# kingjosephm/GAN

Measured on AMD Instinct MI355X. Metric: Pix2Pix train_step images/sec at 256x256, higher is better.
Workload: dtype bf16; 1 GPU; Pix2Pix 256x256 bf16 batch=16/GPU train_step (G fwd, D fwd real+fake, losses, dgrad+wgrad, Adam); global_batch=16, img_size=256, channels=1, parallelism=dp1, hipgraph=True

## Files before the change

gan_amd/csrc/host_util.cpp:

```cpp
#include <nmmintrin.h>
#include <stddef.h>
#include <stdint.h>
#include <string.h>
#include "../../include/gan_amd.h"

extern "C" uint32_t gan_crc32c(uint32_t crc, const void* data, size_t n) {
  const unsigned char* p = (const unsigned char*)data;
  uint64_t c = crc ^ 0xffffffffu;
  while (n && ((uintptr_t)p & 7)) { c = _mm_crc32_u8((uint32_t)c, *p++); --n; }
  while (n >= 8) { uint64_t v; memcpy(&v, p, 8); c = _mm_crc32_u64(c, v); p += 8; n -= 8; }
  while (n) { c = _mm_crc32_u8((uint32_t)c, *p++); --n; }
  return (uint32_t)c ^ 0xffffffffu;
}

#include <atomic>
namespace {
struct Opt { const char* key; std::atomic<int> value; };
Opt g_opts[] = {
    {"conv.big_tiles", {1}},
    {"conv.q128", {55}},
    {"conv.q256n", {80}},
    {"conv.big_min_blocks", {64}},
    {"conv.tall64", {1}},
    {"conv.lean_epilogue", {1}},
    {"conv.tap_share", {7}},
    {"conv.pingpong", {1}},
    {"conv.parity_patch", {1}},
    {"conv.parity_patch_max_n", {64}},
    {"conv.parity_patch_min_blocks", {192}},
    {"conv.split_target", {256}},
    {"conv.split_target_skinny", {1024}},
    {"conv.split_target_big", {256}},
    {"conv.split_target_256", {128}},
    {"conv.split_min_ktiles", {4}},
    {"conv.split_max", {64}},
    {"conv.bwd_fuse_tile", {1}},
    {"conv.stack", {0}},
    {"conv.stack_blocks", {256}},
    {"conv.reduce_stats_rg", {16}},
    {"conv.own_max_kb", {192}},
    {"conv.own_max_rows", {16}},
    {"conv.skn512_min_rows", {0}},
    {"conv.norm_fuse", {1}},
    {"conv.thin_fused", {1}},
    {"conv.thin_k_blocks", {2048}},
    {"conv.thin", {7}},
    {"wgrad.tile256", {0}},
    {"wgrad.pingpong", {1}},
    {"wgrad.row_table", {1}},
    {"wgrad.pingpong_min_rows", {0}},
    {"wgrad.pingpong_128", {1}},
    {"wgrad.pingpong_min_gflop", {30}},
    {"wgrad.split_target", {512}},
    {"wgrad.fold_split_target", {512}},
    {"wgrad.reduce_adam_min_params", {1 << 20}},
    {"wgrad.reduce_adam", {1}},
    {"wgrad.adam_halves_max_rows", {0}},
    {"wgrad.dead_taps", {1}},
    {"norm.fin_in_apply", {0}},
    {"diag.launch_log", {0}},
};
Opt* find_opt(const char* key) {
  if (!key) return nullptr;
  for (Opt& o : g_opts)
    if (!strcmp(o.key, key)) return &o;
  return nullptr;
}
}

int gan_opt(const char* key) {
  Opt* o = find_opt(key);
  return o ? o->value.load(std::memory_order_relaxed) : 0;
}
#include <mutex>
#include <vector>
namespace {
std::atomic<int> g_log_on{0};
std::mutex g_log_mu;
std::vector<const void*> g_log;
}
void gan_launch_note(const void* kernel_host_fn) {
  if (!g_log_on.load(std::memory_order_relaxed)) return;
  std::lock_guard<std::mutex> lk(g_log_mu);
  g_log.push_back(kernel_host_fn);
}
size_t gan_launch_log_ptrs(const void** out, size_t cap) {
  std::lock_guard<std::mutex> lk(g_log_mu);
  for (size_t i = 0; i < g_log.size() && i < cap; ++i) out[i] = g_log[i];
  return g_log.size();
}

extern "C" int gan_set_option(const char* key, int32_t value) {
  Opt* o = find_opt(key);
  if (!o) return GAN_E_ARG;
  o->value.store(value, std::memory_order_relaxed);
  if (!strcmp(key, "diag.launch_log")) {
    std::lock_guard<std::mutex> lk(g_log_mu);
    if (value) g_log.clear();
    g_log_on.store(value ? 1 : 0, std::memory_order_relaxed);
  }
  return 0;
}
extern "C" int gan_get_option(const char* key, int32_t* value) {
  Opt* o = find_opt(key);
  if (!o || !value) return GAN_E_ARG;
  *value = o->value.load(std::memory_order_relaxed);
  return 0;
}
```

gan_amd/csrc/thin.hip:

```cpp
#include "common.h"
#include "conv_params.h"
#include <stdlib.h>
#include <type_traits>

typedef __attribute__((ext_vector_type(8))) short s16x8;
#ifndef THIN_ZS
#define THIN_ZS 20
#endif


struct ThinKParams {
  const void* x; const void* w; void* y; const float* bias;
  int Hs, Ws, xpitch, Hg, Wg, M, S, dy0, dstep, Wrows, ypitch, act, tiles;
  float slope;
  FastDiv divWg, divHg;
};

template <typename T, int ACT>
__global__ __launch_bounds__(256) void conv_thin_k_kernel(const ThinKParams p) {
  const int lane = threadIdx.x & 63, wave = threadIdx.x >> 6;
  const int n = lane & 15, q = lane >> 4;
  const int cbase = blockIdx.y * 64;
  uint4 wf[4][4];
#pragma unroll
  for (int ct = 0; ct < 4; ++ct) {
    const int ch = cbase + (ct >> 1) * 32 + (n >> 2) * 8 + (ct & 1) * 4 + (n & 3);
#pragma unroll
    for (int s = 0; s < 4; ++s) wf[ct][s] = *(const uint4*)((const T*)p.w + ((size_t)(s * 4 + q) * p.Wrows + ch) * 8);
  }
  float bv[2][8];
#pragma unroll
  for (int pr = 0; pr < 2; ++pr)
#pragma unroll
    for (int i = 0; i < 8; ++i) bv[pr][i] = p.bias ? p.bias[cbase + pr * 32 + q * 8 + i] : 0.f;

  for (int tile = blockIdx.x * 4 + wave; tile < p.tiles; tile += gridDim.x * 4) {
    const int m = tile * 16 + n;
    const unsigned t = fdiv((unsigned)m, p.divWg);
    const int gx = m - (int)t * p.Wg;
    const unsigned img = fdiv(t, p.divHg);
    const int gy = (int)t - (int)img * p.Hg;
    const bool rowok = m < p.M;
    const int sx = gx * p.S + p.dy0 + q * p.dstep;
    uint4 xf[4];
#pragma unroll
    for (int s = 0; s < 4; ++s) {
      const int sy = gy * p.S + p.dy0 + s * p.dstep;
      xf[s] = make_uint4(0, 0, 0, 0);
      if (rowok && (unsigned)sy < (unsigned)p.Hs && (unsigned)sx < (unsigned)p.Ws)
        xf[s] = *(const uint4*)((const T*)p.x + ((size_t)(img * p.Hs + sy) * p.Ws + sx) * p.xpitch);
    }
    f32x4 acc[4];
#pragma unroll
    for (int ct = 0; ct < 4; ++ct) {
      acc[ct] = f32x4{0.f, 0.f, 0.f, 0.f};
#pragma unroll
      for (int s = 0; s < 4; ++s) acc[ct] = mma16<T>(wf[ct][s], xf[s], acc[ct]);
    }
    if (rowok) {
      T* yp = (T*)p.y + ((size_t)(img * p.Hg + gy) * p.Wg + gx) * p.ypitch + cbase + q * 8;
#pragma unroll
      for (int pr = 0; pr < 2; ++pr) {
        float v[8];
#pragma unroll
        for (int i = 0; i < 4; ++i) {
          if constexpr (ACT >= 0) {
            v[i] = act_c<ACT>(acc[2 * pr][i] + bv[pr][i], p.slope);
            v[4 + i] = act_c<ACT>(acc[2 * pr + 1][i] + bv[pr][4 + i], p.slope);
          } else {
            v[i] = apply_act(acc[2 * pr][i] + bv[pr][i], p.act, p.slope);
            v[4 + i] = apply_act(acc[2 * pr + 1][i] + bv[pr][4 + i], p.act, p.slope);
          }
        }
        *(uint4*)(yp + pr * 32) = pack16<T>(v);
      }
    }
  }
}

struct ThinNParams {
  const void* x; const void* w; float* z;
  int Mx, xpitch, Cin, Wrows, CO, tiles;
};

template <typename T, int KS>
__global__ __launch_bounds__(256) void conv_thin_n_kernel(const ThinNParams p) {
  extern __shared__ __attribute__((aligned(16))) unsigned char smem[];
  uint4* wl = (uint4*)smem;
  const int lane = threadIdx.x & 63, wave = threadIdx.x >> 6;
  const int n = lane & 15, q = lane >> 4;
  for (int e = threadIdx.x; e < p.CO * KS * 64; e += 256) {
    const int l = e & 63, s = (e >> 6) % KS, c = (e >> 6) / KS;
    wl[e] = *(const uint4*)((const T*)p.w + ((size_t)(l & 15) * p.Wrows + c) * p.Cin + s * 32 + (l >> 4) * 8);
  }
  __syncthreads();
  for (int tile = blockIdx.x * 4 + wave; tile < p.tiles; tile += gridDim.x * 4) {
    const int pix = tile * 16 + n;
    const bool ok = pix < p.Mx;
    uint4 xf[KS];
    const T* xp = (const T*)p.x + (size_t)pix * p.xpitch + q * 8;
#pragma unroll
    for (int s = 0; s < KS; ++s) xf[s] = ok ? *(const uint4*)(xp + s * 32) : make_uint4(0, 0, 0, 0);
    for (int c = 0; c < p.CO; ++c) {
      f32x4 acc = f32x4{0.f, 0.f, 0.f, 0.f};
#pragma unroll
      for (int s = 0; s < KS; ++s) acc = mma16<T>(wl[(c * KS + s) * 64 + lane], xf[s], acc);
      if (ok) *(f32x4*)(p.z + ((size_t)pix * p.CO + c) * 16 + q * 4) = acc;
    }
  }
}

struct Col2imParams {
  const float* z; void* y; const float* bias;
  int Hs, Ws, Ho, Wo, CO, ypitch, out_f32, act, parity, S, dy0, dstep, f16;
  float slope;
  long long total;
  FastDiv divWo, divHo;
};

__global__ __launch_bounds__(256) void conv_thin_col2im_kernel(const Col2imParams p) {
  const long long idx = (long long)blockIdx.x * 256 + threadIdx.x;
  if (idx >= p.total) return;
  const unsigned t = fdiv((unsigned)idx, p.divWo);
  const int X = (int)idx - (int)t * p.Wo;
  const unsigned img = fdiv(t, p.divHo);
  const int Y = (int)t - (int)img * p.Ho;
  int iy[4], ky[4], ix[4], kx[4], ny, nx;
  if (p.parity) {
    ny = nx = 2;
    const int py = Y & 1, gy = Y >> 1, px = X & 1, gx = X >> 1;
#pragma unroll
    for (int a = 0; a < 2; ++a) {
      iy[a] = gy + py - a; ky[a] = 1 - py + 2 * a;
      ix[a] = gx + px - a; kx[a] = 1 - px + 2 * a;
    }
  } else {
    ny = nx = 4;
#pragma unroll
    for (int a = 0; a < 4; ++a) {
      iy[a] = Y * p.S + p.dy0 + a * p.dstep; ky[a] = a;
      ix[a] = X * p.S + p.dy0 + a * p.dstep; kx[a] = a;
    }
  }
  float acc[6] = {0.f, 0.f, 0.f, 0.f, 0.f, 0.f};
  for (int a = 0; a < ny; ++a) {
    if ((unsigned)iy[a] >= (unsigned)p.Hs) continue;
    for (int b = 0; b < nx; ++b) {
      if ((unsigned)ix[b] >= (unsigned)p.Ws) continue;
      const float* zp = p.z + ((size_t)(img * p.Hs + iy[a]) * p.Ws + ix[b]) * p.CO * 16 + ky[a] * 4 + kx[b];
#pragma unroll
      for (int c = 0; c < 6; ++c)
        if (c < p.CO) acc[c] += zp[c * 16];
    }
  }
  const size_t o = ((size_t)(img * p.Ho + Y) * p.Wo + X) * p.ypitch;
#pragma unroll
  for (int c = 0; c < 6; ++c) {
    if (c >= p.CO) break;
    float v = acc[c] + (p.bias ? p.bias[c] : 0.f);
    v = apply_act(v, p.act, p.slope);
    if (p.out_f32) ((float*)p.y)[o + c] = v;
    else if (p.f16) ((f16_t*)p.y)[o + c] = (f16_t)v;
    else ((bf16_t*)p.y)[o + c] = (bf16_t)v;
  }
}

struct ThinNFusedParams {
  const void* x; const void* w; void* y; const float* bias;
  int Hs, Ws, xpitch, Cin, Wrows, CO;
  int Ho, Wo, ypitch, out_f32, act, f16;
  float slope;
  int tilesY, tilesX;
};

template <typename T, int KS, bool PARITY, int TH, int TW>
__global__ __launch_bounds__(256) void conv_thin_n_fused_kernel(const ThinNFusedParams p) {
  constexpr int HB = 1, HA = PARITY ? 1 : 2;
  constexpr int SH = TH + HB + HA, SW = TW + HB + HA, NPX = SH * SW, NT = (NPX + 15) / 16;
  extern __shared__ __attribute__((aligned(16))) unsigned char smem[];
  uint4* wl = (uint4*)smem;
  constexpr int ZS = THIN_ZS;
  float* zl = (float*)(smem + (size_t)p.CO * KS * 1024);
  const int lane = threadIdx.x & 63, wave = threadIdx.x >> 6;
  const int n = lane & 15, q = lane >> 4;
  int b = blockIdx.x;
  const int tx = b % p.tilesX; b /= p.tilesX;
  const int ty = b % p.tilesY; const int img = b / p.tilesY;
  const int y0 = ty * TH - HB, x0 = tx * TW - HB;
  for (int e = threadIdx.x; e < p.CO * KS * 64; e += 256) {
    const int l = e & 63, s = (e >> 6) % KS, c = (e >> 6) / KS;
    wl[e] = *(const uint4*)((const T*)p.w + ((size_t)(l & 15) * p.Wrows + c) * p.Cin + s * 32 + (l >> 4) * 8);
  }
  __syncthreads();
  for (int tile = wave; tile < NT; tile += 4) {
    const int e = tile * 16 + n;
    const int hy = e / SW, hx = e - hy * SW;
    const int sy = y0 + hy, sx = x0 + hx;
    const bool ok = e < NPX && (unsigned)sy < (unsigned)p.Hs && (unsigned)sx < (unsigned)p.Ws;
    uint4 xf[KS];
    const T* xp = (const T*)p.x + ((size_t)(img * p.Hs + sy) * p.Ws + sx) * p.xpitch + q * 8;
#pragma unroll
    for (int s = 0; s < KS; ++s) xf[s] = ok ? *(const uint4*)(xp + s * 32) : make_uint4(0, 0, 0, 0);
    for (int c = 0; c < p.CO; ++c) {
      f32x4 acc = f32x4{0.f, 0.f, 0.f, 0.f};
#pragma unroll
      for (int s = 0; s < KS; ++s) acc = mma16<T>(wl[(c * KS + s) * 64 + lane], xf[s], acc);
      if (e < NPX) *(f32x4*)(zl + ((size_t)c * NPX + e) * ZS + q * 4) = acc;
    }
  }
  __syncthreads();
  auto store = [&](int Y, int X, int c, float v) {
    v += p.bias ? p.bias[c] : 0.f;
    v = apply_act(v, p.act, p.slope);
    const size_t o = ((size_t)(img * p.Ho + Y) * p.Wo + X) * p.ypitch + c;
    if (p.out_f32) ((float*)p.y)[o] = v;
    else if (p.f16) ((f16_t*)p.y)[o] = (f16_t)v;
    else ((bf16_t*)p.y)[o] = (bf16_t)v;
  };
  for (int t = threadIdx.x; t < TH * TW; t += 256) {
    const int ly = t / TW, lx = t - ly * TW;
    const int gy = ty * TH + ly, gx = tx * TW + lx;
    if (PARITY) {
      if (gy >= p.Hs || gx >= p.Ws) continue;
      for (int c = 0; c < p.CO; ++c) {
#pragma unroll
        for (int py = 0; py < 2; ++py)
#pragma unroll
          for (int px = 0; px < 2; ++px) {
            float v = 0.f;
#pragma unroll
            for (int a = 0; a < 2; ++a)
#pragma unroll
              for (int bb = 0; bb < 2; ++bb)
                v += zl[((size_t)c * NPX + (ly + HB + py - a) * SW + (lx + HB + px - bb)) * ZS + (1 - py + 2 * a) * 4 + (1 - px + 2 * bb)];
            store(2 * gy + py, 2 * gx + px, c, v);
          }
      }
    } else {
      if (gy >= p.Ho || gx >= p.Wo) continue;
      for (int c = 0; c < p.CO; ++c) {
        float v = 0.f;
#pragma unroll
        for (int a = 0; a < 4; ++a)
#pragma unroll
          for (int bb = 0; bb < 4; ++bb)
            v += zl[((size_t)c * NPX + (ly + a) * SW + (lx + bb)) * ZS + a * 4 + bb];
        store(gy, gx, c, v);
      }
    }
  }
}

int thin_family(const GanConvDesc* d, int op, const GemmParams& p) {
  const int on = gan_opt("conv.thin"), off = (on & 1) ? (~on & 6) : 1;
  if (off == 1 || d->dtype == GAN_F32) return 0;
  const GanTensor &x = d->x, &y = d->y;
  if (!(off & 2) && y.c <= 6 && (x.c == 64 || x.c == 128 || x.c == 512) && (x.c / 32) * y.c <= 48 &&
      x.pitch % 8 == 0 && ((uintptr_t)x.ptr & 15) == 0 && (p.parity || (p.dstep == 1 && p.dy0 == -1)))
    return 1;
  if (!(off & 4) && !p.parity && x.c == 8 && x.pitch % 8 == 0 && y.c % 64 == 0 && !d->y_f32 && p.vec_store &&
      d->w_rows >= y.c && p.dx0 == p.dy0)
    return 2;
  return 0;
}

static bool thin_n_fused_ok(const GanConvDesc* d, const GemmParams& p) {
  return gan_opt("conv.thin_fused") && d->y.c <= 2 && (p.parity || (p.S == 1 && p.dstep == 1 && p.dy0 == -1 && p.dx0 == -1));
}

size_t thin_workspace_bytes(int family, const GanConvDesc* d, const GemmParams& p) {
  if (family != 1 || thin_n_fused_ok(d, p)) return 0;
  return (size_t)d->x.n * d->x.h * d->x.w * d->y.c * 16 * sizeof(float);
}

int thin_launch(int family, const GanConvDesc* d, const GemmParams& p, hipStream_t st) {
  const GanTensor &x = d->x, &y = d->y;
  if (family == 2) {
    ThinKParams k;
    k.x = p.x; k.w = p.w; k.y = p.y; k.bias = p.bias;
    k.Hs = p.Hs; k.Ws = p.Ws; k.xpitch = p.xpitch; k.Hg = p.Hg; k.Wg = p.Wg; k.M = p.M; k.S = p.S;
    k.dy0 = p.dy0; k.dstep = p.dstep; k.Wrows = p.Wrows; k.ypitch = p.ypitch; k.act = p.act; k.slope = p.slope;
    k.tiles = (p.M + 15) / 16;
    k.divWg = p.divWg; k.divHg = p.divHg;
    const int groups = y.c / 64;
    int gx = (k.tiles + 3) / 4;
    const int capw = gan_opt("conv.thin_k_blocks");
    const int cap = capw / groups > 256 ? capw / groups : 256;
    if (gx > cap) gx = cap;
    const dim3 grid((unsigned)gx, (unsigned)groups);
#define THIN_K(TT)                                                                                              \
    do {                                                                                                        \
      if (k.act == GAN_ACT_NONE) GAN_LAUNCH((conv_thin_k_kernel<TT, GAN_ACT_NONE>), grid, dim3(256), 0, st, k);         \
      else if (k.act == GAN_ACT_LRELU) GAN_LAUNCH((conv_thin_k_kernel<TT, GAN_ACT_LRELU>), grid, dim3(256), 0, st, k);  \
      else GAN_LAUNCH((conv_thin_k_kernel<TT, -1>), grid, dim3(256), 0, st, k);                                 \
    } while (0)
    if (d->dtype == GAN_F16) THIN_K(f16_t); else THIN_K(bf16_t);
#undef THIN_K
    GAN_CHECK_LAUNCH();
    return 0;
  }
  if (family != 1) return GAN_E_ARG;
  if (thin_n_fused_ok(d, p)) {
    ThinNFusedParams f;
    f.x = p.x; f.w = p.w; f.y = p.y; f.bias = p.bias;
    f.Hs = p.Hs; f.Ws = p.Ws; f.xpitch = p.xpitch; f.Cin = x.c; f.Wrows = p.Wrows; f.CO = y.c;
    f.Ho = p.Ho; f.Wo = p.Wo; f.ypitch = p.ypitch; f.out_f32 = p.out_f32; f.act = p.act; f.f16 = d->dtype == GAN_F16; f.slope = p.slope;
    const int KS = x.c / 32;
    auto launch_f = [&](auto* tag, auto parc) -> int {
      typedef typename std::remove_pointer<decltype(tag)>::type T;
      constexpr bool PAR = decltype(parc)::value;
      constexpr int TH = PAR ? 16 : 10, TW = 32;
      constexpr int NPX = (TH + (PAR ? 2 : 3)) * (TW + (PAR ? 2 : 3));
      f.tilesY = ((PAR ? p.Hs : p.Ho) + TH - 1) / TH; f.tilesX = ((PAR ? p.Ws : p.Wo) + TW - 1) / TW;
      const size_t smem = (size_t)f.CO * KS * 1024 + (size_t)NPX * f.CO * THIN_ZS * sizeof(float);
      const dim3 grid((unsigned)(x.n * f.tilesY * f.tilesX));
#define THIN_F(KSV)                                                                                                                  \
      {                                                                                                                               \
        auto kern = conv_thin_n_fused_kernel<T, KSV, PAR, TH, TW>;                                                                    \
        hipError_t e = hipFuncSetAttribute((const void*)kern, hipFuncAttributeMaxDynamicSharedMemorySize, (int)smem);                 \
        if (e != hipSuccess) return (int)e;                                                                                           \
        GAN_LAUNCH(kern, grid, dim3(256), smem, st, f);                                                                       \
      }
      if (KS == 2) THIN_F(2) else if (KS == 4) THIN_F(4) else THIN_F(16)
#undef THIN_F
      GAN_CHECK_LAUNCH();
      return 0;
    };
    if (d->dtype == GAN_F16) return p.parity ? launch_f((f16_t*)nullptr, std::true_type{}) : launch_f((f16_t*)nullptr, std::false_type{});
    return p.parity ? launch_f((bf16_t*)nullptr, std::true_type{}) : launch_f((bf16_t*)nullptr, std::false_type{});
  }
  const size_t zbytes = thin_workspace_bytes(1, d, p);
  if (!d->workspace || d->workspace_bytes < zbytes) return GAN_E_WORKSPACE;
  ThinNParams n;
  n.x = p.x; n.w = p.w; n.z = (float*)d->workspace;
  n.Mx = x.n * x.h * x.w; n.xpitch = p.xpitch; n.Cin = x.c; n.Wrows = p.Wrows; n.CO = y.c;
  n.tiles = (n.Mx + 15) / 16;
  const int KS = x.c / 32;
  int gx = (n.tiles + 3) / 4;
  if (gx > 2048) gx = 2048;
  const size_t smem = (size_t)n.CO * KS * 1024;
  auto launch_n = [&](auto* tag) {
    typedef typename std::remove_pointer<decltype(tag)>::type T;
    if (KS == 2) GAN_LAUNCH((conv_thin_n_kernel<T, 2>), dim3((unsigned)gx), dim3(256), smem, st, n);
    else if (KS == 4) GAN_LAUNCH((conv_thin_n_kernel<T, 4>), dim3((unsigned)gx), dim3(256), smem, st, n);
    else GAN_LAUNCH((conv_thin_n_kernel<T, 16>), dim3((unsigned)gx), dim3(256), smem, st, n);
  };
  if (d->dtype == GAN_F16) launch_n((f16_t*)nullptr); else launch_n((bf16_t*)nullptr);
  GAN_CHECK_LAUNCH();
  Col2imParams c;
  c.z = n.z; c.y = p.y; c.bias = p.bias;
  c.Hs = p.Hs; c.Ws = p.Ws; c.Ho = p.Ho; c.Wo = p.Wo; c.CO = y.c; c.ypitch = p.ypitch; c.out_f32 = p.out_f32;
  c.f16 = d->dtype == GAN_F16;
  c.act = p.act; c.parity = p.parity; c.S = p.S; c.dy0 = p.dy0; c.dstep = p.dstep; c.slope = p.slope;
  c.total = (long long)x.n * p.Ho * p.Wo;
  c.divWo = make_fastdiv((uint32_t)p.Wo); c.divHo = make_fastdiv((uint32_t)p.Ho);
  GAN_LAUNCH(conv_thin_col2im_kernel, dim3((unsigned)((c.total + 255) / 256)), dim3(256), 0, st, c);
  GAN_CHECK_LAUNCH();
  return 0;
}
```

Measured before the change: 5547 images/sec.

## Pipeline input loads and adapt tile size in fused thin-N conv kernel

The fused thin-N conv kernel now takes the output channel count as a compile-time template parameter and stages weight loads through registers. It issues the input-pixel loads for several upcoming tiles ahead of the weight store and barrier, so global-memory latency overlaps with the MFMA work. The host also picks smaller spatial tiles when the default tiling would give fewer than 256 blocks, to fill the GPU on small feature maps. In exchange it uses more registers, which can lower occupancy, and it adds many more kernel instantiations.

Measured after the change: 5558 images/sec (median of 2 runs). About the same (+0.2%).

```diff
diff --git a/gan_amd/csrc/host_util.cpp b/gan_amd/csrc/host_util.cpp
--- a/gan_amd/csrc/host_util.cpp
+++ b/gan_amd/csrc/host_util.cpp
@@ -43,6 +43,7 @@
     {"conv.skn512_min_rows", {0}},
     {"conv.norm_fuse", {1}},
     {"conv.thin_fused", {1}},
+    {"conv.thin_n_tile", {0}},
     {"conv.thin_k_blocks", {2048}},
     {"conv.thin", {7}},
     {"wgrad.tile256", {0}},
diff --git a/gan_amd/csrc/thin.hip b/gan_amd/csrc/thin.hip
--- a/gan_amd/csrc/thin.hip
+++ b/gan_amd/csrc/thin.hip
@@ -1,12 +1,10 @@
 #include "common.h"
 #include "conv_params.h"
+#include "thin_plan.h"
 #include <stdlib.h>
 #include <type_traits>
 
 typedef __attribute__((ext_vector_type(8))) short s16x8;
-#ifndef THIN_ZS
-#define THIN_ZS 20
-#endif
 
 
 struct ThinKParams {
@@ -173,40 +171,69 @@
   int tilesY, tilesX;
 };
 
-template <typename T, int KS, bool PARITY, int TH, int TW>
+template <int KS> struct ThinNDepth { static constexpr int V = KS >= 16 ? 2 : KS >= 4 ? 4 : 6; };
+
+template <typename T, int KS, int CO, bool PARITY, int TH, int TW>
 __global__ __launch_bounds__(256) void conv_thin_n_fused_kernel(const ThinNFusedParams p) {
   constexpr int HB = 1, HA = PARITY ? 1 : 2;
   constexpr int SH = TH + HB + HA, SW = TW + HB + HA, NPX = SH * SW, NT = (NPX + 15) / 16;
+  constexpr int NI = (NT + 3) / 4;
+  constexpr int D = ThinNDepth<KS>::V < NI ? ThinNDepth<KS>::V : NI;
+  constexpr int NW = CO * KS * 64, WI = (NW + 255) / 256;
+  constexpr int ZS = THIN_ZS;
   extern __shared__ __attribute__((aligned(16))) unsigned char smem[];
   uint4* wl = (uint4*)smem;
-  constexpr int ZS = THIN_ZS;
-  float* zl = (float*)(smem + (size_t)p.CO * KS * 1024);
+  float* zl = (float*)(smem + (size_t)CO * KS * 1024);
+
   const int lane = threadIdx.x & 63, wave = threadIdx.x >> 6;
   const int n = lane & 15, q = lane >> 4;
   int b = blockIdx.x;
   const int tx = b % p.tilesX; b /= p.tilesX;
   const int ty = b % p.tilesY; const int img = b / p.tilesY;
   const int y0 = ty * TH - HB, x0 = tx * TW - HB;
-  for (int e = threadIdx.x; e < p.CO * KS * 64; e += 256) {
+  uint4 wr[WI];
+#pragma unroll
+  for (int i = 0; i < WI; ++i) {
+    const int e0 = threadIdx.x + i * 256, e = e0 < NW ? e0 : NW - 1;
     const int l = e & 63, s = (e >> 6) % KS, c = (e >> 6) / KS;
-    wl[e] = *(const uint4*)((const T*)p.w + ((size_t)(l & 15) * p.Wrows + c) * p.Cin + s * 32 + (l >> 4) * 8);
-  }
-  __syncthreads();
-  for (int tile = wave; tile < NT; tile += 4) {
-    const int e = tile * 16 + n;
+    wr[i] = *(const uint4*)((const T*)p.w + ((size_t)(l & 15) * p.Wrows + c) * p.Cin + s * 32 + (l >> 4) * 8);
+  }
+  const T* xsafe = (const T*)p.x + ((size_t)(img * p.Hs + (y0 < 0 ? 0 : y0)) * p.Ws + (x0 < 0 ? 0 : x0)) * p.xpitch + q * 8;
+  uint4 xf[D][KS];
+  auto request = [&](int i, uint4* dst) {
+    const int e = (wave + 4 * i) * 16 + n;
     const int hy = e / SW, hx = e - hy * SW;
     const int sy = y0 + hy, sx = x0 + hx;
     const bool ok = e < NPX && (unsigned)sy < (unsigned)p.Hs && (unsigned)sx < (unsigned)p.Ws;
-    uint4 xf[KS];
-    const T* xp = (const T*)p.x + ((size_t)(img * p.Hs + sy) * p.Ws + sx) * p.xpitch + q * 8;
-#pragma unroll
-    for (int s = 0; s < KS; ++s) xf[s] = ok ? *(const uint4*)(xp + s * 32) : make_uint4(0, 0, 0, 0);
-    for (int c = 0; c < p.CO; ++c) {
+    const T* xp = ok ? (const T*)p.x + ((size_t)(img * p.Hs + sy) * p.Ws + sx) * p.xpitch + q * 8 : xsafe;
+#pragma unroll
+    for (int s = 0; s < KS; ++s) dst[s] = *(const uint4*)(xp + s * 32);
+  };
+#pragma unroll
+  for (int i = 0; i < D; ++i) request(i, xf[i]);
+#pragma unroll
+  for (int i = 0; i < WI; ++i) {
+    const int e0 = threadIdx.x + i * 256;
+    wl[e0 < NW ? e0 : NW - 1] = wr[i];
+  }
+  __syncthreads();
+#pragma unroll
+  for (int i = 0; i < NI; ++i) {
+    const int e = (wave + 4 * i) * 16 + n;
+    const int hy = e / SW, hx = e - hy * SW;
+    const int sy = y0 + hy, sx = x0 + hx;
+    const bool ok = e < NPX && (unsigned)sy < (unsigned)p.Hs && (unsigned)sx < (unsigned)p.Ws;
+    uint4 xv[KS];
+#pragma unroll
+    for (int s = 0; s < KS; ++s) xv[s] = ok ? xf[i % D][s] : make_uint4(0, 0, 0, 0);
+#pragma unroll
+    for (int c = 0; c < CO; ++c) {
       f32x4 acc = f32x4{0.f, 0.f, 0.f, 0.f};
 #pragma unroll
-      for (int s = 0; s < KS; ++s) acc = mma16<T>(wl[(c * KS + s) * 64 + lane], xf[s], acc);
+      for (int s = 0; s < KS; ++s) acc = mma16<T>(wl[(c * KS + s) * 64 + lane], xv[s], acc);
       if (e < NPX) *(f32x4*)(zl + ((size_t)c * NPX + e) * ZS + q * 4) = acc;
     }
+    if (i + D < NI) request(i + D, xf[i % D]);
   }
   __syncthreads();
   auto store = [&](int Y, int X, int c, float v) {
@@ -222,7 +249,7 @@
     const int gy = ty * TH + ly, gx = tx * TW + lx;
     if (PARITY) {
       if (gy >= p.Hs || gx >= p.Ws) continue;
-      for (int c = 0; c < p.CO; ++c) {
+      for (int c = 0; c < CO; ++c) {
 #pragma unroll
         for (int py = 0; py < 2; ++py)
 #pragma unroll
@@ -238,7 +265,7 @@
       }
     } else {
       if (gy >= p.Ho || gx >= p.Wo) continue;
-      for (int c = 0; c < p.CO; ++c) {
+      for (int c = 0; c < CO; ++c) {
         float v = 0.f;
 #pragma unroll
         for (int a = 0; a < 4; ++a)
@@ -306,28 +333,35 @@
     f.Hs = p.Hs; f.Ws = p.Ws; f.xpitch = p.xpitch; f.Cin = x.c; f.Wrows = p.Wrows; f.CO = y.c;
     f.Ho = p.Ho; f.Wo = p.Wo; f.ypitch = p.ypitch; f.out_f32 = p.out_f32; f.act = p.act; f.f16 = d->dtype == GAN_F16; f.slope = p.slope;
     const int KS = x.c / 32;
-    auto launch_f = [&](auto* tag, auto parc) -> int {
-      typedef typename std::remove_pointer<decltype(tag)>::type T;
-      constexpr bool PAR = decltype(parc)::value;
-      constexpr int TH = PAR ? 16 : 10, TW = 32;
-      constexpr int NPX = (TH + (PAR ? 2 : 3)) * (TW + (PAR ? 2 : 3));
-      f.tilesY = ((PAR ? p.Hs : p.Ho) + TH - 1) / TH; f.tilesX = ((PAR ? p.Ws : p.Wo) + TW - 1) / TW;
-      const size_t smem = (size_t)f.CO * KS * 1024 + (size_t)NPX * f.CO * THIN_ZS * sizeof(float);
-      const dim3 grid((unsigned)(x.n * f.tilesY * f.tilesX));
-#define THIN_F(KSV)                                                                                                                  \
-      {                                                                                                                               \
-        auto kern = conv_thin_n_fused_kernel<T, KSV, PAR, TH, TW>;                                                                    \
-        hipError_t e = hipFuncSetAttribute((const void*)kern, hipFuncAttributeMaxDynamicSharedMemorySize, (int)smem);                 \
-        if (e != hipSuccess) return (int)e;                                                                                           \
-        GAN_LAUNCH(kern, grid, dim3(256), smem, st, f);                                                                       \
-      }
-      if (KS == 2) THIN_F(2) else if (KS == 4) THIN_F(4) else THIN_F(16)
+    const bool f16 = d->dtype == GAN_F16;
+    const int gh = p.parity ? p.Hs : p.Ho, gw = p.parity ? p.Ws : p.Wo;
+    const int ti = thin_n_tile_choice(p.parity, gh, gw, x.n, gan_opt("conv.thin_n_tile"));
+    const ThinNTile t = thin_n_tiles(p.parity)[ti];
+    f.tilesY = (gh + t.th - 1) / t.th; f.tilesX = (gw + t.tw - 1) / t.tw;
+    const size_t smem = thin_n_lds_bytes(p.parity, t, f.CO, KS);
+    const dim3 grid((unsigned)thin_n_blocks(t, gh, gw, x.n));
+#define THIN_F(TT, KSV, COV, PAR, TH, TW)                                                                                           \
+    {                                                                                                                             \
+      auto kern = conv_thin_n_fused_kernel<TT, KSV, COV, PAR, TH, TW>;                                                            \
+      hipError_t e = hipFuncSetAttribute((const void*)kern, hipFuncAttributeMaxDynamicSharedMemorySize, (int)smem);               \
+      if (e != hipSuccess) return (int)e;                                                                                         \
+      GAN_LAUNCH(kern, grid, dim3(256), smem, st, f);                                                                             \
+    }
+#define THIN_F_K(TT, COV, PAR, TH, TW)                                                                                              \
+    { if (KS == 2) THIN_F(TT, 2, COV, PAR, TH, TW) else if (KS == 4) THIN_F(TT, 4, COV, PAR, TH, TW) else THIN_F(TT, 16, COV, PAR, TH, TW) }
+#define THIN_F_C(TT, PAR, TH, TW) { if (f.CO == 1) THIN_F_K(TT, 1, PAR, TH, TW) else THIN_F_K(TT, 2, PAR, TH, TW) }
+#define THIN_F_T(PAR, TH, TW) { if (f16) THIN_F_C(f16_t, PAR, TH, TW) else THIN_F_C(bf16_t, PAR, TH, TW) }
+    if (p.parity) {
+      if (ti == 0) THIN_F_T(true, 16, 32) else THIN_F_T(true, 8, 32)
+    } else {
+      if (ti == 0) THIN_F_T(false, 10, 32) else if (ti == 1) THIN_F_T(false, 8, 16) else THIN_F_T(false, 8, 8)
+    }
+#undef THIN_F_T
+#undef THIN_F_C
+#undef THIN_F_K
 #undef THIN_F
-      GAN_CHECK_LAUNCH();
-      return 0;
-    };
-    if (d->dtype == GAN_F16) return p.parity ? launch_f((f16_t*)nullptr, std::true_type{}) : launch_f((f16_t*)nullptr, std::false_type{});
-    return p.parity ? launch_f((bf16_t*)nullptr, std::true_type{}) : launch_f((bf16_t*)nullptr, std::false_type{});
+    GAN_CHECK_LAUNCH();
+    return 0;
   }
   const size_t zbytes = thin_workspace_bytes(1, d, p);
   if (!d->workspace || d->workspace_bytes < zbytes) return GAN_E_WORKSPACE;
diff --git a/gan_amd/csrc/thin_plan.h b/gan_amd/csrc/thin_plan.h
--- /dev/null
+++ b/gan_amd/csrc/thin_plan.h
@@ -0,0 +1,38 @@
+#pragma once
+#include <stddef.h>
+
+#ifndef THIN_ZS
+#define THIN_ZS 20
+#endif
+
+struct ThinNTile { int th, tw; };
+
+static const ThinNTile THIN_N_TILES_PARITY[] = {{16, 32}, {8, 32}};
+static const ThinNTile THIN_N_TILES_S1[] = {{10, 32}, {8, 16}, {8, 8}};
+enum { THIN_N_NTILES_PARITY = 2, THIN_N_NTILES_S1 = 3 };
+
+enum { THIN_N_MIN_BLOCKS = 256 };
+
+static inline int thin_n_ntiles(int parity) { return parity ? THIN_N_NTILES_PARITY : THIN_N_NTILES_S1; }
+static inline const ThinNTile* thin_n_tiles(int parity) { return parity ? THIN_N_TILES_PARITY : THIN_N_TILES_S1; }
+
+static inline long long thin_n_blocks(ThinNTile t, int gridH, int gridW, int images) {
+  return (long long)images * ((gridH + t.th - 1) / t.th) * ((gridW + t.tw - 1) / t.tw);
+}
+
+static inline int thin_n_halo_pixels(int parity, ThinNTile t) {
+  const int h = parity ? 2 : 3;
+  return (t.th + h) * (t.tw + h);
+}
+static inline size_t thin_n_lds_bytes(int parity, ThinNTile t, int CO, int KS) {
+  return (size_t)CO * KS * 1024 + (size_t)thin_n_halo_pixels(parity, t) * CO * THIN_ZS * sizeof(float);
+}
+
+static inline int thin_n_tile_choice(int parity, int gridH, int gridW, int images, int forced) {
+  const int nt = thin_n_ntiles(parity);
+  if (forced > 0) return forced > nt ? nt - 1 : forced - 1;
+  const ThinNTile* t = thin_n_tiles(parity);
+  for (int i = 0; i < nt; ++i)
+    if (thin_n_blocks(t[i], gridH, gridW, images) >= THIN_N_MIN_BLOCKS) return i;
+  return nt - 1;
+}
```
